# usmandroid/80211ParallelEstimation

Measured on AMD Instinct MI355X. Metric: MMSE-estimated 802.11 frames/sec (53 subcarriers) at 1/2/4/8 MI355X; % roofline, higher is better.
Workload: dtype f64; 1 GPU; PS_MMSE textbook, BASELINE configs[2]; frames_per_gpu=65536, global_frames=65536, subcarriers=53, ofdm_blocks=15, parallelism=dp1 (frames sharded, 1 RCCL state broadcast)

## Files before the change

### 80211parallelestimation_amd/csrc/wce_api.cpp

```cpp
#include <hip/hip_runtime.h>
#include <cstdio>
#include <cstring>
#include <map>
#include <memory>
#include <mutex>
#include <new>
#include <string>
#include <vector>

#include "wce_internal.h"

using wce::State;

struct wce_ctx {
    int device = 0;
    State *d_state = nullptr;
    bool ready = false;
    bool has_host = false;
    State host;
    int32_t mode = -1;
    bool fuse = true;
    bool bdot = true;
    int32_t cov_k0 = -1;
    int32_t cov_rank = 0;
    int cov_taps = 0;
    int cov_path = 0;
    int cus = 0;
    bool r1_plain = false;
    bool cm_on = false;
    bool cm_use = true;
    std::vector<wce_complex> rhh;
    std::mutex ws_mu;
    std::map<void *, std::unique_ptr<wce::Workspace>> ws_by_stream;
    int64_t ws_hint = 0;
};

static constexpr int64_t WS_LD = 64;
static constexpr int64_t WS_ARRAYS = 5;

static thread_local std::string g_err;

static bool state_r1_plain(const State *st) { return st->acoef == 1.0 && st->xmask == (1ull << wce::NSC) - 1; }

static int fail(int code, const char *what)
{
    g_err = what;
    return code;
}

static int hipfail(hipError_t e, const char *what)
{
    g_err = std::string(what) + ": " + hipGetErrorString(e);
    return WCE_EHIP;
}

#define HIPCHECK(x, what)                         \
    do {                                          \
        hipError_t e_ = (x);                      \
        if (e_ != hipSuccess) return hipfail(e_, what); \
    } while (0)
// ... 14 lines not shown
struct DeviceGuard {
    int prev = -1;
    explicit DeviceGuard(int d)
    {
        if (hipGetDevice(&prev) != hipSuccess) prev = -1;
        if (prev != d) (void)hipSetDevice(d);
    }
    ~DeviceGuard()
    {
        int cur = -1;
        if (prev >= 0 && hipGetDevice(&cur) == hipSuccess && cur != prev) (void)hipSetDevice(prev);
    }
};
}

extern "C" {

const char *wce_last_error(void) { return g_err.c_str(); }
const char *wce_version(void) { return "wce 0.1.0 (gfx950)"; }

int wce_ctx_create_empty(wce_ctx **out, int device)
{
    if (!out) return fail(WCE_EINVAL, "null ctx pointer");
    int rc = check_device(device);
    if (rc) return rc;
    wce_ctx *c = new (std::nothrow) wce_ctx();
    if (!c) return fail(WCE_ENOMEM, "ctx alloc");
    c->device = device;
    DeviceGuard g(device);
    if (hipDeviceGetAttribute(&c->cus, hipDeviceAttributeMultiprocessorCount, device) != hipSuccess || c->cus <= 0) {
        delete c;
        return fail(WCE_EHIP, "hipDeviceGetAttribute(multiprocessor count)");
    }
    hipError_t e = hipMalloc(&c->d_state, sizeof(State));
    if (e != hipSuccess) { delete c; return hipfail(e, "hipMalloc(state)"); }
    e = hipMemset(c->d_state, 0, sizeof(State));
    if (e != hipSuccess) { (void)hipFree(c->d_state); delete c; return hipfail(e, "hipMemset(state)"); }
    *out = c;
    return WCE_OK;
}

int wce_ctx_create(wce_ctx **out, int device, const wce_complex *tx_pre, const wce_complex *rx_pre, double ow2,
                   int mode)
{
    if (!out || !tx_pre || !rx_pre) return fail(WCE_EINVAL, "null argument");
    if (mode != WCE_MMSE_REF && mode != WCE_MMSE_TEXTBOOK) return fail(WCE_EINVAL, "bad mmse mode");
    if (!(ow2 > 0)) return fail(WCE_EINVAL, "ow2 must be > 0");
    wce_ctx *c = nullptr;
    int rc = wce_ctx_create_empty(&c, device);
    if (rc) return rc;
    wce::ldc txl[wce::NSC], rxl[wce::NSC], hlt[wce::NSC];
    for (int k = 0; k < wce::NSC; k++) {
        txl[k].re = tx_pre[k].re; txl[k].im = tx_pre[k].im;
        rxl[k].re = rx_pre[k].re; rxl[k].im = rx_pre[k].im;
    }
    wce::host_lt_ls(txl, rxl, hlt);
    rc = wce::host_build_state(&c->host, wce::host_reference_F(), wce::host_reference_invF(), hlt, txl, ow2, mode);
    if (rc) { wce_ctx_destroy(c); return fail(rc, "state build"); }
    c->has_host = true;
    c->mode = mode;
    c->r1_plain = state_r1_plain(&c->host);
    DeviceGuard g(device);
    hipError_t e = hipMemcpy(c->d_state, &c->host, sizeof(State), hipMemcpyHostToDevice);
    if (e != hipSuccess) { wce_ctx_destroy(c); return hipfail(e, "upload state"); }
    c->ready = true;
    *out = c;
// ... 501 lines not shown
    if (r.prep != wce::FcPrep::None) {
        rc = prep_frame_cov(c, in, out, r, sa, ws, stream);
        if (rc) return rc;
    }
    double *aux = ws ? ws + (WS_ARRAYS - 1) * n * WS_LD * 2 : nullptr;
    if (split) {
        sa.split = 1;
        if (r.form == wce::SolveForm::Bordered) {
            sa.dots = aux;
        } else {
            sa.w = ws;
            sa.ws = WS_LD;
        }
    }
    double *H = reinterpret_cast<double *>(out->ps_mmse);
    if (r.cm) {
        uint8_t *flags = reinterpret_cast<uint8_t *>(aux);
        rc = wce::launch_cm(c->d_state, sa, flags, stream);
        if (rc) return fail(rc, "constant-modulus launch");
        sa.skip = flags;
    }
    const State *st = c->d_state;
    switch (r.solve) {
    case wce::SolveStep::None: return WCE_OK;
    case wce::SolveStep::RefLsElemDone:
        rc = wce::launch_ref_ls_elem(st, sa, la, true, stream);
        return rc ? fail(rc, "ls epilogue launch") : WCE_OK;
    case wce::SolveStep::LowRank:
        rc = wce::launch_mmse_lr(st, cov_lr_k0(c), c->cov_rank, c->cov_taps, sa, stream);
        if (rc) return fail(rc, "mmse_lr launch");
        break;
    case wce::SolveStep::RefPilots: rc = wce::launch_mmse_ref_pilots(st, sa, stream); break;
    case wce::SolveStep::RefLsElem: rc = wce::launch_ref_ls_elem(st, sa, la, false, stream); break;
    case wce::SolveStep::Closed: rc = wce::launch_mmse_rank1(st, sa, false, c->cus, c->r1_plain, stream); break;
    case wce::SolveStep::ClosedNt: rc = wce::launch_mmse_rank1(st, sa, true, c->cus, c->r1_plain, stream); break;
    case wce::SolveStep::Factor: rc = wce::launch_mmse_factor(st, sa, r.form, stream); break;
    case wce::SolveStep::Fused: rc = wce::launch_mmse_solve_ls(st, sa, la, r.form, stream); break;
    }
    if (rc) return fail(rc, "mmse_solve launch");
    switch (r.finish) {
    case wce::Finish::None: break;
    case wce::Finish::AvgBlocks:
        rc = wce::launch_avg_blocks(ws, WS_LD, H, out->out_stride, n, stream);
        return rc ? fail(rc, "block average launch") : WCE_OK;
    case wce::Finish::FcFinish: rc = wce::launch_fc_finish(sa, aux, H, out->out_stride, stream); break;
    case wce::Finish::MatvecAvg:
        rc = wce::launch_matvec_avg(st->C, ws, WS_LD, sa.nblk, H, out->out_stride, n, stream);
        break;
    case wce::Finish::Apply:
        rc = wce::launch_mmse_apply(st, H, H, out->out_stride, n, stream, sa.skip);
        break;
    }
    return rc ? fail(rc, "mmse apply launch") : WCE_OK;
}

int wce_estimate(wce_ctx *c, const wce_frames *in, const wce_outputs *out, uint32_t mask, void *stream)
{
    return estimate_impl(c, in, out, mask, stream, nullptr);
}

int wce_estimate_noise(wce_ctx *c, const wce_frames *in, const wce_outputs *out, uint32_t mask, const double *ow2,
                       void *stream)
{
    return estimate_impl(c, in, out, mask, stream, nullptr, ow2);
}

struct wce_plan {
    wce_plan() = default;
// ... 535 lines not shown
```

### 80211parallelestimation_amd/csrc/wce_internal.h

```cpp
#pragma once
#include <mutex>
#include <stdint.h>
#include <stddef.h>
#include "../../include/wce.h"
#include "wce_route.h"

namespace wce {

constexpr int NSC = WCE_NSC;
constexpr int NBLK = WCE_NBLK;
constexpr int NPAD = 64;
constexpr int CLD = 64;
constexpr int PILOT[4] = {WCE_P0, WCE_P1, WCE_P2, WCE_P3};
constexpr int32_t STATE_MAGIC = 0x80211;
constexpr int32_t STATE_LAYOUT = 9;
constexpr int COV_K0_MAX = 6;

constexpr int LRL_RMAX = 8;
constexpr int LRL_NP = LRL_RMAX * (LRL_RMAX + 1) / 2;
struct State {
    double C[CLD * CLD * 2];
    double Mu[CLD * CLD * 2];
    double Wp[4 * NPAD * 2];
    double cvec[NPAD * 2];
// ... 145 lines not shown

struct ViterbiArgs {
    const float *llr;
    int64_t lfs, lbs, n;
    int32_t mod, rate, T;
    uint32_t flags;
    uint8_t *bits;
    const uint8_t *ref;
    uint32_t *nbiterr;
    int64_t bits_stride, ref_stride;
};

struct ReencodeArgs {
    const uint8_t *bits;
    const double *theta;
    const double *ptx, *rx;
    int64_t bits_stride, fs, bs, n;
    int32_t mod, rate;
    double scale, d;
    double *tx, *h;
    int64_t tfs, tbs, hs;
};

int launch_ls(const State *st, const LsArgs &a, void *stream);
int launch_demod(const DemodArgs &a, void *stream);
int launch_demap(const DemapArgs &a, void *stream);
int launch_reencode(const ReencodeArgs &a, void *stream);
int launch_viterbi(const ViterbiArgs &a, void *stream);
int decode_info_bits(int mod, int rate);
int launch_front(const FrontArgs &a, bool preamble, void *stream);
int launch_sync(const SyncArgs &a, int cus, void *stream);
int launch_mmse_ref_pilots(const State *st, const SolveArgs &a, void *stream);
int launch_mmse_factor(const State *st, const SolveArgs &a, SolveForm form, void *stream);
int launch_mmse_rank1(const State *st, const SolveArgs &a, bool nt, int cus, bool plain, void *stream);
int rank1_rows_per_sweep(int cus);
int launch_mmse_solve_ls(const State *st, const SolveArgs &a, const LsArgs &l, SolveForm form, void *stream);
int launch_ref_ls_elem(const State *st, const SolveArgs &a, const LsArgs &l, bool mmse_done, void *stream);
int launch_mmse_apply(const State *st, const double *W, double *H, int64_t stride, int64_t n, void *stream,
                      const uint8_t *skip = nullptr);
int launch_cm(const State *st, const SolveArgs &a, uint8_t *flags, void *stream);
int launch_matvec(const double *M1, const double *M2, const double *X, int64_t xs, double *Y1, double *Y2,
                  int64_t ys, int64_t n, bool qin, void *stream);
int launch_matvec_avg(const double *M, const double *X, int64_t xs, int nb, double *Y, int64_t ys, int64_t n,
                      void *stream);
int launch_fc_finish(const SolveArgs &a, const double *dots, double *H, int64_t hs, void *stream);
int launch_synth(const State *st, const SynthArgs &a, void *stream);
int launch_lr_quad2(const State *st, int rank, const SolveArgs &a, void *stream, int form = 0);
int launch_mmse_lr(const State *st, int k0, int rank, int taps, const SolveArgs &a, void *stream);
const char *lr_kernel_name(int k0, int rank, int taps, int64_t units);
int launch_ref_fc(const State *st, const SolveArgs &a, const double *rx_pre, int64_t ps, const double *tx_pre,
                  void *stream);
int launch_fc_u(const State *st, const double *rx_pre, int64_t ps, const double *tx_pre, double *U, int64_t us,
                int64_t n, void *stream);
int launch_ref_w(const State *st, const double *X, int64_t xs, double *W, int64_t ws, int64_t n, void *stream);
int launch_avg_blocks(const double *X, int64_t xs, double *H, int64_t hs, int64_t n, void *stream);
int set_flat_chunk(int64_t frames);
constexpr int WCE_VARIANT_REF = 0;
constexpr int WCE_VARIANT_LS = 1;
constexpr int WCE_VARIANT_REF_LS = 2;
constexpr int WCE_VARIANT_LR = 3;
constexpr int WCE_VARIANT_REF_FC = 4;
constexpr int WCE_VARIANT_R1 = 5;
constexpr int WCE_VARIANT_COUNT = 6;
int variant_value(int which);
int set_variant(int which, int value);
int launch_ldc_convert(const void *src, void *dst, int64_t n, bool to_complex, void *stream);
int launch_nonfinite_scan(const double *H, int64_t stride, int64_t n, bool f32, uint32_t *bits,
// ... 14 lines not shown
```

### 80211parallelestimation_amd/csrc/wce_kernels.hip

```cpp
#include <hip/hip_runtime.h>
#include "wce_internal.h"
#include "wce_device.h"

namespace wce {

constexpr int LS_WAVES = 4;
constexpr int LS_FRAMES = 4;

struct LsLane {
    double2 tpk, tden, hlt_shared;
    double cq, s0, s1, s2, s3, alpha, dk0, dk1, dk2;
    int seg;
};
__device__ __forceinline__ LsLane ls_lane(const State *__restrict__ st, const double *tx_pre, int k)
{
    LsLane c;
    const double *txp = tx_pre ? tx_pre : st->tx_pre;
    c.tpk = ld2(txp, k);
    c.cq = c.tpk.x - c.tpk.y;
    c.tden = make_double2(c.cq * c.tpk.x, c.cq * c.tpk.y);
    c.hlt_shared = ld2(st->h_lt, k);
    c.s0 = st->sinc[0][k]; c.s1 = st->sinc[1][k]; c.s2 = st->sinc[2][k]; c.s3 = st->sinc[3][k];
    c.seg = k < WCE_P1 ? 0 : (k < WCE_P2 ? 1 : 2);
    c.alpha = (double)(k - (c.seg == 0 ? WCE_P0 : (c.seg == 1 ? WCE_P1 : WCE_P2))) * (1.0 / 14.0);
// ... 2320 lines not shown
                                                             unsigned long long *n_bad)
{
    const uint32_t E = nfr * (uint32_t)NSC;
    for (uint32_t e = blockIdx.x * 256u + threadIdx.x; e < E; e += gridDim.x * 256u) {
        const uint32_t f = e / NSC, k = e - f * NSC;
        const int64_t idx = (f_begin + f) * stride + k;
        double re, im;
        if constexpr (F32) {
            const v2f t = reinterpret_cast<const v2f *>(H)[idx];
            re = t.x;
            im = t.y;
        } else {
            const double2 t = ld2(H, idx);
            re = t.x;
            im = t.y;
        }
        if (!(__builtin_isfinite(re) && __builtin_isfinite(im))) {
            const int64_t fg = f_begin + f;
            const uint32_t bit = 1u << (fg & 31);
            const uint32_t old = atomicOr(&bits[fg >> 5], bit);
            if (!(old & bit) && n_bad) atomicAdd(n_bad, 1ull);
        }
    }
}

static int hip_status(hipError_t e) { return e == hipSuccess ? WCE_OK : WCE_EHIP; }

constexpr int LR_FPW = 64;
constexpr int64_t LR_FPW_BELOW = 131072;
constexpr int64_t LR_STAGE_FROM = 0;
static int g_variant[WCE_VARIANT_COUNT] = {0, 2, 0, 0, 0, 0};
int set_variant(int which, int value)
{
    if (which < 0 || which >= WCE_VARIANT_COUNT || value < 0 || value > 15) return WCE_EINVAL;
    __atomic_store_n(&g_variant[which], value, __ATOMIC_RELAXED);
    return WCE_OK;
}
static inline int variant(int which) { return __atomic_load_n(&g_variant[which], __ATOMIC_RELAXED); }
int variant_value(int which) { return which >= 0 && which < WCE_VARIANT_COUNT ? variant(which) : 0; }

static int cu_count()
{
    constexpr int kMaxDev = 64;
    static int cache[kMaxDev] = {};
    int dev = 0;
    if (hipGetDevice(&dev) != hipSuccess || dev < 0) dev = 0;
    int *slot = dev < kMaxDev ? &cache[dev] : nullptr;
    int cus = slot ? __atomic_load_n(slot, __ATOMIC_RELAXED) : 0;
    if (cus <= 0) {
        int n = 0;
        cus = hipDeviceGetAttribute(&n, hipDeviceAttributeMultiprocessorCount, dev) == hipSuccess && n > 0 ? n : 256;
        if (slot) __atomic_store_n(slot, cus, __ATOMIC_RELAXED);
    }
    return cus;
}

static int64_t tile_blocks(int64_t tiles, int waves_per_cu)
{
    const int64_t cap = (int64_t)cu_count() * waves_per_cu / LS_WAVES;
    const int64_t need = (tiles + LS_WAVES - 1) / LS_WAVES;
    return need < cap ? need : cap;
}

int launch_ls(const State *st, const LsArgs &a, void *stream)
{
    if (a.n <= 0) return WCE_OK;
    const int64_t groups = (a.n + LS_FRAMES - 1) / LS_FRAMES;
// ... 774 lines not shown
```

### 80211parallelestimation_amd/csrc/wce_rank1.hip

```cpp
#include "wce_internal.h"
#include "wce_device.h"

namespace wce {

__device__ __forceinline__ double2 r1_mul(double2 a, double2 b)
{
#pragma clang fp contract(off)
    return make_double2(a.x * b.x - a.y * b.y, a.x * b.y + a.y * b.x);
}
__device__ __forceinline__ double2 r1_add(double2 a, double2 b)
{
#pragma clang fp contract(off)
    return make_double2(a.x + b.x, a.y + b.y);
}

__device__ __forceinline__ double2 rank1_p(double2 u, double2 w, bool cwg)
{
#pragma clang fp contract(off)
    return cwg ? r1_mul(w, u) : make_double2(u.x * u.x + u.y * u.y, 0.0);
}

template <bool PLAIN>
__device__ __forceinline__ double2 rank1_s(const double2 (&x)[4], const double2 (&r)[4], const double2 (&u)[4],
                                           const double2 (&w)[4], const double2 (&p)[4], bool cwg, double ac,
                                           double bc)
{
#pragma clang fp contract(off)
    double2 g = make_double2(0.0, 0.0), q = g;
#pragma unroll
    for (int m = 0; m < 4; ++m) {
        const double x2 = x[m].x * x[m].x + x[m].y * x[m].y;
        const double ax2 = PLAIN ? x2 : ac * x2;
        const double2 gk = make_double2(ax2 * p[m].x, ax2 * p[m].y);
        const double2 qk = r1_mul(r1_mul(w[m], cconj(x[m])), r[m]);
        g = m ? r1_add(g, gk) : gk;
        q = m ? r1_add(q, qk) : qk;
    }
    g = row16_sum(g);
    q = row16_sum(q);
    const double2 d = make_double2(bc + g.x, g.y);
    double2 t;
    if (cwg) {
        const double den = d.x * d.x + d.y * d.y;
        t = make_double2((q.x * d.x + q.y * d.y) / den, (q.y * d.x - q.x * d.y) / den);
    } else {
        t = make_double2(q.x / d.x, q.y / d.x);
    }
    double2 c = make_double2(0.0, 0.0);
#pragma unroll
    for (int m = 0; m < 4; ++m) {
        const double2 xu = r1_mul(x[m], u[m]);
        const double2 at = r1_mul(PLAIN ? xu : make_double2(ac * xu.x, ac * xu.y), t);
        const double2 rho = make_double2(r[m].x - at.x, r[m].y - at.y);
        const double ti = 2.0 * x[m].y;
        const double2 ck = r1_mul(w[m], make_double2(-(ti * rho.y), ti * rho.x));
        c = m ? r1_add(c, ck) : ck;
    }
    c = row16_sum(c);
    return make_double2(t.x + c.x / bc, t.y + c.y / bc);
}

constexpr int R1_WG_PER_CU = 4;
constexpr int R1_POL_DEFAULT = 0, R1_POL_NT = 1, R1_POL_NT_STORES = 2, R1_POL_NT_LOADS = 3;
constexpr int R1_POL_U_FIRST = 4;
constexpr int R1_POL_TX_FIRST = 5;

constexpr bool r1_prefetch(bool noise, bool shared) { return shared && !noise; }

template <int POL, bool NOISE, bool SHARED, bool SPLIT, bool PF, bool PLAIN>
__global__ __launch_bounds__(256, R1_WG_PER_CU) void mmse_rank1_kernel(const State *__restrict__ st, SolveArgs a)
{
    static_assert(!PF || r1_prefetch(NOISE, SHARED), "this instantiation has no registers for a second unit");
    constexpr bool NTL = POL == R1_POL_NT || POL == R1_POL_NT_LOADS;
    constexpr bool NTS = POL == R1_POL_NT || POL == R1_POL_NT_STORES;
    constexpr bool LF = POL != R1_POL_U_FIRST;
    constexpr bool TXF = POL == R1_POL_TX_FIRST;
    static_assert(!TXF || (SHARED && PLAIN), "the tx-first order is built for the shared-u builds without mask and scale");
    const int i = threadIdx.x & 15;
    const uint32_t rpw = blockDim.x >> 4;
    int64_t n = a.n;
    if (LF) {
        auto held = [](int64_t &c, auto v) __attribute__((always_inline)) { asm("" : "+s"(c) : "s"(v)); };
        held(n, st), held(n, a.tx), held(n, a.rx), held(n, a.fs), held(n, a.bs), held(n, a.blk), held(n, a.cu);
        held(n, rpw), held(n, gridDim.x);
        if (SPLIT) held(n, a.nblk), held(n, a.dots);
        else held(n, a.w), held(n, a.ws);
        if (NOISE) held(n, a.ow2);
        if (!SHARED) held(n, a.cs), held(n, a.cw);
    }
    const uint32_t units = (uint32_t)(SPLIT ? n * a.nblk : n);
    const uint32_t rows = gridDim.x * rpw;
    uint32_t g = blockIdx.x * rpw + (threadIdx.x >> 4);
    if (g >= units) return;
    const bool cwg = !SHARED && a.cw != nullptr;
    double ac;
    uint64_t xm;
    auto scalars = [&](double &b) __attribute__((always_inline)) {
        ac = PLAIN ? 1.0 : st->acoef;
        xm = PLAIN ? ~0ull : st->xmask;
        if (!NOISE) b = st->bcoef;
    };
    const double2 zero = make_double2(0.0, 0.0);
    auto lane_again = [](int l) __attribute__((always_inline)) {
        asm volatile("" : "+v"(l));
        return l;
    };
    auto frame_of = [&](uint32_t gu) __attribute__((always_inline)) { return SPLIT ? gu / (uint32_t)a.nblk : gu; };
    auto fetch = [&](uint32_t gu, double2(&xl)[4], double2(&rl)[4], double &bc, int part = 0) __attribute__((always_inline)) {
        const uint32_t f = frame_of(gu);
        const int b = SPLIT ? (int)(gu - f * (uint32_t)a.nblk) : 0;
        const int64_t base = (int64_t)f * a.fs + (int64_t)(a.blk + b) * a.bs + lane_again(i);
        if (TXF) {
            if (part != 2) {
#pragma unroll
                for (int m = 0; m < 3; ++m) xl[m] = ld2(a.tx, base + 16 * m);
                xl[3] = zero;
                if (i < NSC - 48) xl[3] = ld2(a.tx, base + 48);
            }
            if (part != 1) {
#pragma unroll
                for (int m = 0; m < 3; ++m) rl[m] = ld2(a.rx, base + 16 * m);
                rl[3] = zero;
                if (i < NSC - 48) rl[3] = ld2(a.rx, base + 48);
                if (NOISE) bc = a.ow2[f];
            }
            return;
        }
#pragma unroll
        for (int m = 0; m < 3; ++m) {
            xl[m] = NTL ? ld2_nt(a.tx, base + 16 * m) : ld2(a.tx, base + 16 * m);
            rl[m] = NTL ? ld2_nt(a.rx, base + 16 * m) : ld2(a.rx, base + 16 * m);
        }
        xl[3] = zero;
        rl[3] = zero;
        if (i < NSC - 48) {
            xl[3] = NTL ? ld2_nt(a.tx, base + 48) : ld2(a.tx, base + 48);
            rl[3] = NTL ? ld2_nt(a.rx, base + 48) : ld2(a.rx, base + 48);
        }
        if (NOISE) bc = a.ow2[f];
    };
    auto factors = [&](int64_t cb, double2(&u)[4], double2(&w)[4], double2(&p)[4]) __attribute__((always_inline)) {
        const int64_t ub = cb + i;
        const bool live = i < NSC - 48;
        if (SHARED) {
#pragma unroll
            for (int m = 0; m < 3; ++m) {
                u[m] = ld2(a.cu, ub + 16 * m);
                w[m] = cconj(u[m]);
            }
            u[3] = zero;
            w[3] = zero;
            if (live) {
                u[3] = ld2(a.cu, ub + 48);
                w[3] = cconj(u[3]);
            }
        } else {
#pragma unroll
            for (int m = 0; m < 3; ++m) u[m] = ld2(a.cu, ub + 16 * m);
            u[3] = zero;
            if (live) u[3] = ld2(a.cu, ub + 48);
            if (cwg) {
#pragma unroll
                for (int m = 0; m < 3; ++m) w[m] = ld2(a.cw, ub + 16 * m);
                w[3] = zero;
                if (live) w[3] = ld2(a.cw, ub + 48);
            } else {
#pragma unroll
                for (int m = 0; m < 3; ++m) w[m] = cconj(u[m]);
                w[3] = live ? cconj(u[3]) : zero;
            }
        }
#pragma unroll
        for (int m = 0; m < 4; ++m) p[m] = rank1_p(u[m], w[m], cwg);
    };
    double2 u[4], w[4], p[4];
    double2 xc[4], rc[4], xn[4], rn[4];
    double bc = 0.0, bn;
    scalars(bc);
    if (TXF) {
        fetch(g, xc, rc, bc, 1);
#pragma unroll
        for (int m = 0; m < 3; ++m) u[m] = ld2(a.cu, i + 16 * m);
        u[3] = zero;
        if (i < NSC - 48) u[3] = ld2(a.cu, i + 48);
        fetch(g, xc, rc, bc, 2);
#pragma unroll
        for (int m = 0; m < 4; ++m) {
            w[m] = m < 3 || i < NSC - 48 ? cconj(u[m]) : zero;
            p[m] = rank1_p(u[m], w[m], cwg);
        }
    } else {
        if (LF) fetch(g, xc, rc, bc);
        if (SHARED) factors(0, u, w, p);
    }
    bn = bc;
    auto trip = [&](double2(&xc)[4], double2(&rc)[4], double &bc, double2(&xn)[4], double2(&rn)[4], double &bn)
                    __attribute__((always_inline)) {
        if (!PF && !LF) fetch(g, xc, rc, bc);
        const uint32_t f = frame_of(g);
        if (!SHARED) factors((int64_t)f * a.cs, u, w, p);
        const bool more = g + rows < units;
        if (PF && more) fetch(g + rows, xn, rn, bn);
        double2 x[4];
#pragma unroll
        for (int m = 0; m < 4; ++m)
            x[m] = PLAIN || ((xm >> ((i + 16 * m) & 63)) & 1ull) ? xc[m] : zero;
        double2 pl[4];
#pragma unroll
        for (int m = 0; m < 4; ++m) {
            double2 um = u[m];
            if (PF) asm volatile("" : "+v"(um.x), "+v"(um.y));
            pl[m] = PF ? rank1_p(um, w[m], cwg) : p[m];
        }
        double2 s = rank1_s<PLAIN>(x, rc, u, w, pl, cwg, ac, bc);
        if (NOISE && !(bc > 0.0 && bc < __builtin_inf())) s = make_double2(__builtin_nan(""), __builtin_nan(""));
        if (SPLIT) {
            if (i == 0) st2(a.dots, g, s);
// ... 35 lines not shown
    dim3 g, b;
    bool pf;
};

template <int POL, bool NOISE, bool SHARED, bool PLAIN>
static void launch_r1_split(const State *st, const SolveArgs &a, const R1Shape &h, hipStream_t s)
{
    if constexpr (r1_prefetch(NOISE, SHARED)) {
        if (h.pf) {
            if (a.split) hipLaunchKernelGGL((mmse_rank1_kernel<POL, NOISE, SHARED, true, true, PLAIN>), h.g, h.b, 0, s, st, a);
            else hipLaunchKernelGGL((mmse_rank1_kernel<POL, NOISE, SHARED, false, true, PLAIN>), h.g, h.b, 0, s, st, a);
            return;
        }
    }
    if (a.split) hipLaunchKernelGGL((mmse_rank1_kernel<POL, NOISE, SHARED, true, false, PLAIN>), h.g, h.b, 0, s, st, a);
    else hipLaunchKernelGGL((mmse_rank1_kernel<POL, NOISE, SHARED, false, false, PLAIN>), h.g, h.b, 0, s, st, a);
}
template <int POL, bool PLAIN = false>
static void launch_r1_pol(const State *st, const SolveArgs &a, const R1Shape &h, hipStream_t s)
{
    const bool shared = a.cs == 0 && !a.cw;
    if constexpr (POL == R1_POL_TX_FIRST) {
        if (a.ow2) launch_r1_split<POL, true, true, PLAIN>(st, a, h, s);
        else launch_r1_split<POL, false, true, PLAIN>(st, a, h, s);
    } else if (a.ow2) {
        if (shared) launch_r1_split<POL, true, true, PLAIN>(st, a, h, s);
        else launch_r1_split<POL, true, false, PLAIN>(st, a, h, s);
    } else {
        if (shared) launch_r1_split<POL, false, true, PLAIN>(st, a, h, s);
        else launch_r1_split<POL, false, false, PLAIN>(st, a, h, s);
    }
}

int launch_mmse_rank1(const State *st, const SolveArgs &a, bool nt, int cus, bool plain, void *stream)
{
    if (!a.cu) return WCE_EINVAL;
    if (a.split ? !a.dots : !a.w) return WCE_EINVAL;
    if (a.n <= 0) return WCE_OK;
    if (a.nblk > 1 && !a.split) return WCE_EINVAL;
    if (a.ow2 && a.cw) return WCE_EINVAL;
    const int64_t units = a.split ? a.n * a.nblk : a.n;
    if (units > 0x7fffffffll) return WCE_EINVAL;
    const int shape = variant_value(WCE_VARIANT_R1);
    const int rpw = shape == 8 ? 4 : shape == 9 ? 8 : 16;
    int64_t wgs = (units + rpw - 1) / rpw;
    const bool looping = shape == 4 || shape == 7;
    const int64_t cap = shape == 4 ? 3 : shape == 7 ? rank1_rows_per_sweep(cus) / 16 : wgs;
    if (wgs > cap) wgs = cap;
    const R1Shape h{dim3((unsigned)wgs), dim3(16u * rpw), looping};
    hipStream_t s = (hipStream_t)stream;
    if (nt) launch_r1_pol<R1_POL_NT>(st, a, h, s);
    else if (shape == 5) launch_r1_pol<R1_POL_NT_STORES>(st, a, h, s);
    else if (shape == 6) launch_r1_pol<R1_POL_NT_LOADS>(st, a, h, s);
    else if (shape == 10) launch_r1_pol<R1_POL_U_FIRST>(st, a, h, s);
    else if (!plain || shape == 11) launch_r1_pol<R1_POL_DEFAULT>(st, a, h, s);
    else if (a.cs == 0 && !a.cw && shape != 12) launch_r1_pol<R1_POL_TX_FIRST, true>(st, a, h, s);
    else launch_r1_pol<R1_POL_DEFAULT, true>(st, a, h, s);
    return hipGetLastError() == hipSuccess ? WCE_OK : WCE_EHIP;
}

}
```

### 80211parallelestimation_amd/csrc/wce_route.cpp

```cpp
#include <cstring>
#include <string>

#include "wce_internal.h"
#include "wce_route.h"
#include "../../include/wce_debug.h"

namespace wce {

int check_route_facts(const RouteFacts &f)
{
    if (f.mode != WCE_MMSE_REF && f.mode != WCE_MMSE_TEXTBOOK && f.mode != WCE_MMSE_COV) return WCE_EINVAL;
    if (f.semantics != WCE_SEM_C && f.semantics != WCE_SEM_MATLAB) return WCE_EINVAL;
    if (f.mask & ~0x7Fu) return WCE_EINVAL;
    if ((f.mask & WCE_MMSE_FRAME_COV) && !(f.mask & WCE_EST_PS_MMSE)) return WCE_EINVAL;
    if (f.mode != WCE_MMSE_COV && (f.lr_k0 >= 0 || f.cm)) return WCE_EINVAL;
    if (f.noise && (f.mode != WCE_MMSE_TEXTBOOK || !(f.mask & WCE_EST_PS_MMSE))) return WCE_EINVAL;
    return WCE_OK;
}

Route plan_route(const RouteFacts &f)
{
    Route r;
    const bool ls = (f.mask & (WCE_EST_LS_ALL | WCE_EQUALIZE)) != 0;
    const bool mmse = (f.mask & WCE_EST_PS_MMSE) != 0;
// ... 50 lines not shown
    case FcPrep::None: break;
    case FcPrep::RefFc: add("ref_fc"); break;
    case FcPrep::FcU: add("fc_u"); break;
    case FcPrep::General:
        if (!r.fc_lt_ready) add("ls");
        add("matvec");
        if (r.fc_ref_w) add("ref_w");
        break;
    }
    if (r.cm) add("cm");
    switch (r.solve) {
    case SolveStep::None: break;
    case SolveStep::RefPilots: add("ref_pilots"); break;
    case SolveStep::RefLsElem: add("ref_ls_elem"); break;
    case SolveStep::RefLsElemDone: add("ref_ls_elem_done"); break;
    case SolveStep::Closed: add("mmse_rank1"); break;
    case SolveStep::ClosedNt: add("mmse_rank1_nt"); break;
    case SolveStep::Factor: add(std::string("factor_") + form[(int)r.form]); break;
    case SolveStep::Fused: add(std::string("fused_") + form[(int)r.form]); break;
    case SolveStep::LowRank: add("mmse_lr"); break;
    }
    switch (r.finish) {
    case Finish::None: break;
    case Finish::FcFinish: add("fc_finish"); break;
    case Finish::MatvecAvg: add("matvec_avg"); break;
    case Finish::Apply: add("apply"); break;
    case Finish::AvgBlocks: add("avg_blocks"); break;
    }
    if (s.size() + 1 > cap || !buf) return -1;
    std::memcpy(buf, s.c_str(), s.size() + 1);
    return (int)s.size();
}

}

extern "C" int wce_debug_route(int mode, int bdot, int fuse, int cm, int lr_k0, int cov_rank, int semantics,
                               unsigned mask, int ls_f32, int r1, int ref_fc, int ref_ls, char *buf, size_t cap)
{
    const wce::RouteFacts f{mode, bdot != 0, fuse != 0, cm != 0, lr_k0, cov_rank, semantics, mask, ls_f32 != 0, r1, ref_fc, ref_ls};
    if (wce::check_route_facts(f)) return WCE_EINVAL;
    return wce::route_names(wce::plan_route(f), buf, cap) < 0 ? WCE_EINVAL : WCE_OK;
}

extern "C" int wce_debug_route_noise(int mode, int bdot, int fuse, int cm, int lr_k0, int cov_rank, int semantics,
                                     unsigned mask, int ls_f32, int r1, int ref_fc, int ref_ls, int noise, char *buf,
                                     size_t cap)
{
    wce::RouteFacts f{mode, bdot != 0, fuse != 0, cm != 0, lr_k0, cov_rank, semantics, mask, ls_f32 != 0, r1, ref_fc, ref_ls};
    f.noise = noise != 0;
    if (wce::check_route_facts(f)) return WCE_EINVAL;
    return wce::route_names(wce::plan_route(f), buf, cap) < 0 ? WCE_EINVAL : WCE_OK;
}
```

### 80211parallelestimation_amd/csrc/wce_route.h

```cpp
#pragma once
#include <cstddef>
#include <cstdint>

namespace wce {

struct RouteFacts {
    int mode;
    bool bdot;
    bool fuse;
    bool cm;
    int lr_k0;
    int cov_rank;
    int semantics;
    uint32_t mask;
    bool ls_f32;
    int r1, ref_fc, ref_ls;
    bool noise;
};

enum class FcPrep : uint8_t {
    None,
    RefFc,
    FcU,
    General,
// ... 5 lines not shown
    Dense,
};

enum class SolveStep : uint8_t {
    None,
    RefPilots,
    RefLsElem,
    RefLsElemDone,
    Closed,
    ClosedNt,
    Factor,
    Fused,
    LowRank,
};

enum class Finish : uint8_t { None, FcFinish, MatvecAvg, Apply, AvgBlocks };

struct Route {
    bool ls_pass = false;
    FcPrep prep = FcPrep::None;
    bool fc_lt_ready = false;
    bool fc_ref_w = false;
    bool cm = false;
    SolveStep solve = SolveStep::None;
    SolveForm form = SolveForm::Dense;
    Finish finish = Finish::None;
    bool workspace = false;
};

int check_route_facts(const RouteFacts &f);
Route plan_route(const RouteFacts &f);
int route_names(const Route &r, char *buf, size_t cap);

}
```

### 80211parallelestimation_amd/wce.py

```python
from __future__ import annotations

import ctypes
import os
from ctypes import POINTER, byref, c_double, c_int, c_int32, c_int64, c_size_t, c_uint32, c_uint64, c_void_p

import numpy as np

NSC = 53
NBLK = 15
DC = 26
PILOTS = (5, 19, 33, 47)

LT_LS = 1 << 0
PS_LINEAR = 1 << 1
PS_CUBIC = 1 << 2
PS_SINC = 1 << 3
PS_MMSE = 1 << 4
EQUALIZE = 1 << 5
LS_ALL = 0xF
ALL = 0x3F
OUT_LS_F32 = 1
FRAME_COV = 1 << 6

MMSE_REF = 0
# ... 55 lines not shown
    _fields_ = [("eq", c_void_p), ("sym", c_void_p), ("theta", c_void_p), ("evm", c_void_p), ("nerr", c_void_p),
                ("eq_frame_stride", c_int64), ("eq_block_stride", c_int64), ("sym_frame_stride", c_int64),
                ("sym_block_stride", c_int64)]


class ReencodePar(ctypes.Structure):
    _fields_ = [("bits", c_void_p), ("bits_stride", c_int64), ("modulation", c_int32), ("rate", c_int32),
                ("scale", c_double), ("theta", c_void_p)]


class ReencodeOut(ctypes.Structure):
    _fields_ = [("tx", c_void_p), ("tx_frame_stride", c_int64), ("tx_block_stride", c_int64), ("h", c_void_p),
                ("h_stride", c_int64)]


_lib = None

ABI = {
    "wce_ctx_create": [POINTER(c_void_p), c_int, c_void_p, c_void_p, c_double, c_int],
    "wce_ctx_create_empty": [POINTER(c_void_p), c_int],
    "wce_ctx_destroy": [c_void_p],
    "wce_ctx_reserve": [c_void_p, c_int64],
    "wce_ctx_reserve_stream": [c_void_p, c_int64, c_void_p],
    "wce_plan_create": [POINTER(c_void_p), c_void_p, c_void_p, c_void_p, c_uint32],
    "wce_plan_launch": [c_void_p, c_void_p],
    "wce_plan_destroy": [c_void_p],
    "wce_ctx_create_cov": [POINTER(c_void_p), c_int, c_void_p, c_void_p, c_void_p, c_double],
    "wce_state_build_cov": [c_void_p, c_size_t, c_void_p, c_void_p, c_void_p, c_double],
    "wce_debug_set_fusion": [c_void_p, c_int],
    "wce_debug_set_border_dot": [c_void_p, c_int],
    "wce_debug_set_flat_chunk": [ctypes.c_int64],
    "wce_debug_set_variant": [c_int, c_int],
    "wce_debug_rank1_rows_per_sweep": [c_void_p],
    "wce_debug_set_cov_path": [c_void_p, c_int],
    "wce_debug_lr_kernel": [c_void_p, c_int64],
    "wce_debug_route": [c_int] * 7 + [c_uint32] + [c_int] * 4 + [ctypes.c_char_p, c_size_t],
    "wce_debug_route_noise": [c_int] * 7 + [c_uint32] + [c_int] * 5 + [ctypes.c_char_p, c_size_t],
    "wce_debug_cov_factor": [c_void_p, c_size_t, c_void_p, POINTER(c_int), POINTER(c_int), POINTER(c_double),
                             POINTER(c_double)],
    "wce_ctx_cov_info": [c_void_p, POINTER(c_int), POINTER(c_int), POINTER(c_double), POINTER(c_double)],
    "wce_ctx_set_modulus": [c_void_p, c_void_p],
    "wce_state_set_modulus": [c_void_p, c_size_t, c_void_p, c_void_p],
    "wce_debug_set_cm": [c_void_p, c_int],
    "wce_debug_compat_state_builds": [],
    "wce_ctx_state": [c_void_p, POINTER(c_void_p), POINTER(c_size_t)],
    "wce_ctx_mark_ready": [c_void_p],
    "wce_state_size": [],
    "wce_state_build": [c_void_p, c_size_t, c_void_p, c_void_p, c_double, c_int],
    "wce_ctx_load_state": [c_void_p, c_void_p, c_size_t],
    "wce_state_validate": [c_void_p, c_size_t, POINTER(c_int)],
    "wce_ctx_get_shared": [c_void_p, c_void_p, c_void_p, POINTER(c_double), POINTER(c_double)],
    "wce_estimate": [c_void_p, POINTER(Frames), POINTER(Outputs), c_uint32, c_void_p],
    "wce_estimate_noise": [c_void_p, POINTER(Frames), POINTER(Outputs), c_uint32, c_void_p, c_void_p],
    "wce_mmse_solve": [c_void_p, POINTER(Frames), c_void_p, c_int64, c_void_p],
    "wce_mmse_apply": [c_void_p, c_void_p, c_void_p, c_int64, c_int64, c_void_p],
    "wce_synth_frames": [c_void_p, c_void_p, c_void_p, c_void_p, c_int64, c_int64, c_int64, c_int64, c_int64,
                         c_uint64, c_void_p, c_double, c_double, c_void_p],
    "wce_front_end_blocks": [c_void_p, c_void_p, c_int64, c_int64, c_int32, c_void_p, c_int64, c_int64, c_void_p],
    "wce_front_end_preamble": [c_void_p, c_void_p, c_int64, c_int64, c_int64, c_void_p, c_int64, c_void_p,
                               c_void_p],
    "wce_front_end_blocks_cfo": [c_void_p, c_void_p, c_int64, c_int64, c_int32, c_void_p, c_int64, c_void_p, c_int64,
                                 c_int64, c_void_p],
    "wce_front_end_preamble_cfo": [c_void_p, c_void_p, c_int64, c_int64, c_int64, c_void_p, c_int64, c_void_p,
                                   c_void_p, c_int, c_void_p],
    "wce_front_end_sync": [c_void_p, c_void_p, c_int64, c_int64, c_int64, c_void_p, c_double, c_int32, c_void_p,
                           c_void_p, c_void_p],
# ... 857 lines not shown
```

### include/wce_debug.h

```cpp
#ifndef WCE_DEBUG_H
#define WCE_DEBUG_H
#include <stddef.h>
#ifdef __cplusplus
extern "C" {
#endif
int wce_debug_reference_F(long double *out);
int wce_debug_reference_invF(long double *out);
int wce_debug_build_state(const double *tx_pre, const double *rx_pre, double ow2, int mode, double *C,
                          double *h_lt, double *sinc, double *ab, unsigned long long *xmask);
int wce_debug_cov_factor(const void *blob, size_t bytes, double *U, int *rank, int *k0, double *lmax, double *lmin);
struct wce_ctx;
int wce_debug_set_fusion(struct wce_ctx *ctx, int on);
int wce_debug_set_border_dot(struct wce_ctx *ctx, int on);
int wce_debug_set_flat_chunk(long long frames);
int wce_debug_set_variant(int which, int value);
int wce_debug_rank1_rows_per_sweep(struct wce_ctx *ctx);
int wce_debug_route(int mode, int bdot, int fuse, int cm, int lr_k0, int cov_rank, int semantics, unsigned mask,
                    int ls_f32, int r1, int ref_fc, int ref_ls, char *buf, size_t cap);
int wce_debug_route_noise(int mode, int bdot, int fuse, int cm, int lr_k0, int cov_rank, int semantics,
                          unsigned mask, int ls_f32, int r1, int ref_fc, int ref_ls, int noise, char *buf,
                          size_t cap);
int wce_debug_set_cov_path(struct wce_ctx *ctx, int path);
const char *wce_debug_lr_kernel(struct wce_ctx *ctx, long long units);
int wce_debug_set_cm(struct wce_ctx *ctx, int on);
unsigned long long wce_debug_compat_state_builds(void);
#ifdef __cplusplus
}
#endif
#endif
```

Measured before the change: 2.302 billion frames/s.

## Add specialized rank-1 MMSE head kernel with XCD-aware workgroup remapping

New measurement: 2.376 billion frames/s (median of 6 runs). 3.2% higher.

```diff
diff --git a/80211parallelestimation_amd/csrc/wce_api.cpp b/80211parallelestimation_amd/csrc/wce_api.cpp
--- a/80211parallelestimation_amd/csrc/wce_api.cpp
+++ b/80211parallelestimation_amd/csrc/wce_api.cpp
@@ -26,6 +26,7 @@
     int cov_taps = 0;
     int cov_path = 0;
     int cus = 0;
+    int xcds = 1;
     bool r1_plain = false;
     bool cm_on = false;
     bool cm_use = true;
@@ -106,6 +107,12 @@
         delete c;
         return fail(WCE_EHIP, "hipDeviceGetAttribute(multiprocessor count)");
     }
+    hipDeviceProp_t prop;
+    if (hipGetDeviceProperties(&prop, device) != hipSuccess) {
+        delete c;
+        return fail(WCE_EHIP, "hipGetDeviceProperties");
+    }
+    c->xcds = std::strncmp(prop.gcnArchName, "gfx950", 6) == 0 ? wce::R1_HEAD_XCDS : 1;
     hipError_t e = hipMalloc(&c->d_state, sizeof(State));
     if (e != hipSuccess) { delete c; return hipfail(e, "hipMalloc(state)"); }
     e = hipMemset(c->d_state, 0, sizeof(State));
@@ -673,8 +680,8 @@
         break;
     case wce::SolveStep::RefPilots: rc = wce::launch_mmse_ref_pilots(st, sa, stream); break;
     case wce::SolveStep::RefLsElem: rc = wce::launch_ref_ls_elem(st, sa, la, false, stream); break;
-    case wce::SolveStep::Closed: rc = wce::launch_mmse_rank1(st, sa, false, c->cus, c->r1_plain, stream); break;
-    case wce::SolveStep::ClosedNt: rc = wce::launch_mmse_rank1(st, sa, true, c->cus, c->r1_plain, stream); break;
+    case wce::SolveStep::Closed: rc = wce::launch_mmse_rank1(st, sa, false, c->cus, c->xcds, c->r1_plain, stream); break;
+    case wce::SolveStep::ClosedNt: rc = wce::launch_mmse_rank1(st, sa, true, c->cus, c->xcds, c->r1_plain, stream); break;
     case wce::SolveStep::Factor: rc = wce::launch_mmse_factor(st, sa, r.form, stream); break;
     case wce::SolveStep::Fused: rc = wce::launch_mmse_solve_ls(st, sa, la, r.form, stream); break;
     }
diff --git a/80211parallelestimation_amd/csrc/wce_internal.h b/80211parallelestimation_amd/csrc/wce_internal.h
--- a/80211parallelestimation_amd/csrc/wce_internal.h
+++ b/80211parallelestimation_amd/csrc/wce_internal.h
@@ -201,7 +201,7 @@
 int launch_sync(const SyncArgs &a, int cus, void *stream);
 int launch_mmse_ref_pilots(const State *st, const SolveArgs &a, void *stream);
 int launch_mmse_factor(const State *st, const SolveArgs &a, SolveForm form, void *stream);
-int launch_mmse_rank1(const State *st, const SolveArgs &a, bool nt, int cus, bool plain, void *stream);
+int launch_mmse_rank1(const State *st, const SolveArgs &a, bool nt, int cus, int nx, bool plain, void *stream);
 int rank1_rows_per_sweep(int cus);
 int launch_mmse_solve_ls(const State *st, const SolveArgs &a, const LsArgs &l, SolveForm form, void *stream);
 int launch_ref_ls_elem(const State *st, const SolveArgs &a, const LsArgs &l, bool mmse_done, void *stream);
diff --git a/80211parallelestimation_amd/csrc/wce_kernels.hip b/80211parallelestimation_amd/csrc/wce_kernels.hip
--- a/80211parallelestimation_amd/csrc/wce_kernels.hip
+++ b/80211parallelestimation_amd/csrc/wce_kernels.hip
@@ -2376,7 +2376,7 @@
 static int g_variant[WCE_VARIANT_COUNT] = {0, 2, 0, 0, 0, 0};
 int set_variant(int which, int value)
 {
-    if (which < 0 || which >= WCE_VARIANT_COUNT || value < 0 || value > 15) return WCE_EINVAL;
+    if (which < 0 || which >= WCE_VARIANT_COUNT || value < 0 || value > 31) return WCE_EINVAL;
     __atomic_store_n(&g_variant[which], value, __ATOMIC_RELAXED);
     return WCE_OK;
 }
diff --git a/80211parallelestimation_amd/csrc/wce_rank1.hip b/80211parallelestimation_amd/csrc/wce_rank1.hip
--- a/80211parallelestimation_amd/csrc/wce_rank1.hip
+++ b/80211parallelestimation_amd/csrc/wce_rank1.hip
@@ -1,66 +1,7 @@
-#include "wce_internal.h"
-#include "wce_device.h"
+#include "wce_rank1_body.h"
 
 namespace wce {
 
-__device__ __forceinline__ double2 r1_mul(double2 a, double2 b)
-{
-#pragma clang fp contract(off)
-    return make_double2(a.x * b.x - a.y * b.y, a.x * b.y + a.y * b.x);
-}
-__device__ __forceinline__ double2 r1_add(double2 a, double2 b)
-{
-#pragma clang fp contract(off)
-    return make_double2(a.x + b.x, a.y + b.y);
-}
-
-__device__ __forceinline__ double2 rank1_p(double2 u, double2 w, bool cwg)
-{
-#pragma clang fp contract(off)
-    return cwg ? r1_mul(w, u) : make_double2(u.x * u.x + u.y * u.y, 0.0);
-}
-
-template <bool PLAIN>
-__device__ __forceinline__ double2 rank1_s(const double2 (&x)[4], const double2 (&r)[4], const double2 (&u)[4],
-                                           const double2 (&w)[4], const double2 (&p)[4], bool cwg, double ac,
-                                           double bc)
-{
-#pragma clang fp contract(off)
-    double2 g = make_double2(0.0, 0.0), q = g;
-#pragma unroll
-    for (int m = 0; m < 4; ++m) {
-        const double x2 = x[m].x * x[m].x + x[m].y * x[m].y;
-        const double ax2 = PLAIN ? x2 : ac * x2;
-        const double2 gk = make_double2(ax2 * p[m].x, ax2 * p[m].y);
-        const double2 qk = r1_mul(r1_mul(w[m], cconj(x[m])), r[m]);
-        g = m ? r1_add(g, gk) : gk;
-        q = m ? r1_add(q, qk) : qk;
-    }
-    g = row16_sum(g);
-    q = row16_sum(q);
-    const double2 d = make_double2(bc + g.x, g.y);
-    double2 t;
-    if (cwg) {
-        const double den = d.x * d.x + d.y * d.y;
-        t = make_double2((q.x * d.x + q.y * d.y) / den, (q.y * d.x - q.x * d.y) / den);
-    } else {
-        t = make_double2(q.x / d.x, q.y / d.x);
-    }
-    double2 c = make_double2(0.0, 0.0);
-#pragma unroll
-    for (int m = 0; m < 4; ++m) {
-        const double2 xu = r1_mul(x[m], u[m]);
-        const double2 at = r1_mul(PLAIN ? xu : make_double2(ac * xu.x, ac * xu.y), t);
-        const double2 rho = make_double2(r[m].x - at.x, r[m].y - at.y);
-        const double ti = 2.0 * x[m].y;
-        const double2 ck = r1_mul(w[m], make_double2(-(ti * rho.y), ti * rho.x));
-        c = m ? r1_add(c, ck) : ck;
-    }
-    c = row16_sum(c);
-    return make_double2(t.x + c.x / bc, t.y + c.y / bc);
-}
-
-constexpr int R1_WG_PER_CU = 4;
 constexpr int R1_POL_DEFAULT = 0, R1_POL_NT = 1, R1_POL_NT_STORES = 2, R1_POL_NT_LOADS = 3;
 constexpr int R1_POL_U_FIRST = 4;
 constexpr int R1_POL_TX_FIRST = 5;
@@ -111,17 +52,9 @@
         const int b = SPLIT ? (int)(gu - f * (uint32_t)a.nblk) : 0;
         const int64_t base = (int64_t)f * a.fs + (int64_t)(a.blk + b) * a.bs + lane_again(i);
         if (TXF) {
-            if (part != 2) {
-#pragma unroll
-                for (int m = 0; m < 3; ++m) xl[m] = ld2(a.tx, base + 16 * m);
-                xl[3] = zero;
-                if (i < NSC - 48) xl[3] = ld2(a.tx, base + 48);
-            }
+            if (part != 2) r1_fetch_row(a.tx, base, i, xl);
             if (part != 1) {
-#pragma unroll
-                for (int m = 0; m < 3; ++m) rl[m] = ld2(a.rx, base + 16 * m);
-                rl[3] = zero;
-                if (i < NSC - 48) rl[3] = ld2(a.rx, base + 48);
+                r1_fetch_row(a.rx, base, i, rl);
                 if (NOISE) bc = a.ow2[f];
             }
             return;
@@ -179,10 +112,7 @@
     scalars(bc);
     if (TXF) {
         fetch(g, xc, rc, bc, 1);
-#pragma unroll
-        for (int m = 0; m < 3; ++m) u[m] = ld2(a.cu, i + 16 * m);
-        u[3] = zero;
-        if (i < NSC - 48) u[3] = ld2(a.cu, i + 48);
+        r1_fetch_row(a.cu, i, i, u);
         fetch(g, xc, rc, bc, 2);
 #pragma unroll
         for (int m = 0; m < 4; ++m) {
@@ -284,7 +214,9 @@
     }
 }
 
-int launch_mmse_rank1(const State *st, const SolveArgs &a, bool nt, int cus, bool plain, void *stream)
+void launch_mmse_rank1_head(const State *st, const SolveArgs &a, const R1HeadShape &h, void *stream);
+
+int launch_mmse_rank1(const State *st, const SolveArgs &a, bool nt, int cus, int nx, bool plain, void *stream)
 {
     if (!a.cu) return WCE_EINVAL;
     if (a.split ? !a.dots : !a.w) return WCE_EINVAL;
@@ -294,6 +226,12 @@
     const int64_t units = a.split ? a.n * a.nblk : a.n;
     if (units > 0x7fffffffll) return WCE_EINVAL;
     const int shape = variant_value(WCE_VARIANT_R1);
+    const R1HeadShape head = rank1_head_shape(
+        R1HeadFacts{a.cs == 0 && !a.cw, a.split != 0, a.ow2 != nullptr, a.cw != nullptr, plain, nt, shape, a.fs, a.ws, a.n}, nx);
+    if (head.threads) {
+        launch_mmse_rank1_head(st, a, head, stream);
+        return hipGetLastError() == hipSuccess ? WCE_OK : WCE_EHIP;
+    }
     const int rpw = shape == 8 ? 4 : shape == 9 ? 8 : 16;
     int64_t wgs = (units + rpw - 1) / rpw;
     const bool looping = shape == 4 || shape == 7;
diff --git a/80211parallelestimation_amd/csrc/wce_rank1_body.h b/80211parallelestimation_amd/csrc/wce_rank1_body.h
--- /dev/null
+++ b/80211parallelestimation_amd/csrc/wce_rank1_body.h
@@ -0,0 +1,74 @@
+#pragma once
+#include "wce_internal.h"
+#include "wce_device.h"
+
+namespace wce {
+
+__device__ __forceinline__ double2 r1_mul(double2 a, double2 b)
+{
+#pragma clang fp contract(off)
+    return make_double2(a.x * b.x - a.y * b.y, a.x * b.y + a.y * b.x);
+}
+__device__ __forceinline__ double2 r1_add(double2 a, double2 b)
+{
+#pragma clang fp contract(off)
+    return make_double2(a.x + b.x, a.y + b.y);
+}
+
+__device__ __forceinline__ double2 rank1_p(double2 u, double2 w, bool cwg)
+{
+#pragma clang fp contract(off)
+    return cwg ? r1_mul(w, u) : make_double2(u.x * u.x + u.y * u.y, 0.0);
+}
+
+template <bool PLAIN>
+__device__ __forceinline__ double2 rank1_s(const double2 (&x)[4], const double2 (&r)[4], const double2 (&u)[4],
+                                           const double2 (&w)[4], const double2 (&p)[4], bool cwg, double ac,
+                                           double bc)
+{
+#pragma clang fp contract(off)
+    double2 g = make_double2(0.0, 0.0), q = g;
+#pragma unroll
+    for (int m = 0; m < 4; ++m) {
+        const double x2 = x[m].x * x[m].x + x[m].y * x[m].y;
+        const double ax2 = PLAIN ? x2 : ac * x2;
+        const double2 gk = make_double2(ax2 * p[m].x, ax2 * p[m].y);
+        const double2 qk = r1_mul(r1_mul(w[m], cconj(x[m])), r[m]);
+        g = m ? r1_add(g, gk) : gk;
+        q = m ? r1_add(q, qk) : qk;
+    }
+    g = row16_sum(g);
+    q = row16_sum(q);
+    const double2 d = make_double2(bc + g.x, g.y);
+    double2 t;
+    if (cwg) {
+        const double den = d.x * d.x + d.y * d.y;
+        t = make_double2((q.x * d.x + q.y * d.y) / den, (q.y * d.x - q.x * d.y) / den);
+    } else {
+        t = make_double2(q.x / d.x, q.y / d.x);
+    }
+    double2 c = make_double2(0.0, 0.0);
+#pragma unroll
+    for (int m = 0; m < 4; ++m) {
+        const double2 xu = r1_mul(x[m], u[m]);
+        const double2 at = r1_mul(PLAIN ? xu : make_double2(ac * xu.x, ac * xu.y), t);
+        const double2 rho = make_double2(r[m].x - at.x, r[m].y - at.y);
+        const double ti = 2.0 * x[m].y;
+        const double2 ck = r1_mul(w[m], make_double2(-(ti * rho.y), ti * rho.x));
+        c = m ? r1_add(c, ck) : ck;
+    }
+    c = row16_sum(c);
+    return make_double2(t.x + c.x / bc, t.y + c.y / bc);
+}
+
+__device__ __forceinline__ void r1_fetch_row(const double *p, int64_t base, int i, double2 (&v)[4])
+{
+#pragma unroll
+    for (int m = 0; m < 3; ++m) v[m] = ld2(p, base + 16 * m);
+    v[3] = make_double2(0.0, 0.0);
+    if (i < NSC - 48) v[3] = ld2(p, base + 48);
+}
+
+constexpr int R1_WG_PER_CU = 4;
+
+}
diff --git a/80211parallelestimation_amd/csrc/wce_rank1_head.hip b/80211parallelestimation_amd/csrc/wce_rank1_head.hip
--- /dev/null
+++ b/80211parallelestimation_amd/csrc/wce_rank1_head.hip
@@ -0,0 +1,66 @@
+#include "wce_rank1_body.h"
+
+namespace wce {
+
+template <int T, bool XCD8>
+__global__ __launch_bounds__(T, R1_WG_PER_CU) void mmse_rank1_head_kernel(const State *st, const double *tx,
+                                                                          const double *rx, const double *cu,
+                                                                          double *H, uint32_t n, uint32_t fs,
+                                                                          uint32_t ws)
+{
+    static_assert(T == 64 || T == 128 || T == 256, "whole waves, at most mmse_rank1_kernel's workgroup");
+    constexpr uint32_t RPW = T / 16;
+    const int i = threadIdx.x & 15;
+    constexpr uint32_t NX = R1_HEAD_XCDS;
+    uint32_t wg = blockIdx.x;
+    if (XCD8) {
+        const uint32_t groups = (n + RPW - 1) / RPW;
+        wg = rank1_head_group(wg, NX, (groups + NX - 1) / NX);
+        if (wg >= groups) return;
+    }
+    const uint32_t g = wg * RPW + (threadIdx.x >> 4);
+    if (g >= n) return;
+    const double bc = st->bcoef;
+    double2 x[4], r[4], u[4], w[4], p[4];
+    const int64_t base = (int64_t)((uint64_t)g * fs) + i;
+    r1_fetch_row(tx, base, i, x);
+    r1_fetch_row(cu, i, i, u);
+    r1_fetch_row(rx, base, i, r);
+#pragma unroll
+    for (int m = 0; m < 4; ++m) {
+        w[m] = m < 3 || i < NSC - 48 ? cconj(u[m]) : make_double2(0.0, 0.0);
+        p[m] = rank1_p(u[m], w[m], false);
+    }
+    const double2 s = rank1_s<true>(x, r, u, w, p, false, 1.0, bc);
+    const int64_t hb = (int64_t)((uint64_t)g * ws) + i;
+#pragma unroll
+    for (int m = 0; m < 4; ++m)
+        if (i + 16 * m < NSC) st2(H, hb + 16 * m, r1_mul(u[m], s));
+}
+
+template <int T>
+static void launch_head(const State *st, const SolveArgs &a, bool remap, hipStream_t s)
+{
+    constexpr int64_t RPW = T / 16;
+    const int64_t groups = (a.n + RPW - 1) / RPW;
+    const double *tx = a.tx + 2 * ((int64_t)a.blk * a.bs), *rx = a.rx + 2 * ((int64_t)a.blk * a.bs);
+    const uint32_t n = (uint32_t)a.n, fs = (uint32_t)a.fs, ws = (uint32_t)a.ws;
+    if (remap) {
+        const int64_t per = (groups + R1_HEAD_XCDS - 1) / R1_HEAD_XCDS;
+        hipLaunchKernelGGL((mmse_rank1_head_kernel<T, true>), dim3((unsigned)(R1_HEAD_XCDS * per)), dim3(T), 0, s, st, tx, rx,
+                           a.cu, a.w, n, fs, ws);
+    } else {
+        hipLaunchKernelGGL((mmse_rank1_head_kernel<T, false>), dim3((unsigned)groups), dim3(T), 0, s, st, tx, rx,
+                           a.cu, a.w, n, fs, ws);
+    }
+}
+
+void launch_mmse_rank1_head(const State *st, const SolveArgs &a, const R1HeadShape &h, void *stream)
+{
+    hipStream_t s = (hipStream_t)stream;
+    if (h.threads == 64) launch_head<64>(st, a, h.remap, s);
+    else if (h.threads == 128) launch_head<128>(st, a, h.remap, s);
+    else launch_head<256>(st, a, h.remap, s);
+}
+
+}
diff --git a/80211parallelestimation_amd/csrc/wce_route.cpp b/80211parallelestimation_amd/csrc/wce_route.cpp
--- a/80211parallelestimation_amd/csrc/wce_route.cpp
+++ b/80211parallelestimation_amd/csrc/wce_route.cpp
@@ -106,6 +106,35 @@
     return (int)s.size();
 }
 
+R1HeadShape rank1_head_shape(const R1HeadFacts &f, int nx)
+{
+    const R1HeadShape old{0, false};
+    if (!f.shared || f.split || f.noise || f.cw || !f.plain || f.nt) return old;
+    if (f.fs < 0 || f.fs > 0xffffffffll || f.ws < 0 || f.ws > 0xffffffffll || f.n > 0x7fffffffll) return old;
+    const int v = f.variant == 0 ? R1_VARIANT_ADOPTED : f.variant;
+    if (v < R1_VARIANT_HEAD_FIRST || v > R1_VARIANT_HEAD_LAST) return old;
+    const int k = (v - R1_VARIANT_HEAD_FIRST) % 3;
+    return R1HeadShape{64 << k, v >= R1_VARIANT_HEAD_FIRST + 3 && nx == R1_HEAD_XCDS};
+}
+
+}
+
+extern "C" int wce_debug_rank1_head(int shared, int split, int noise, int cw, int plain, int nt, int variant,
+                                    long long fs, long long ws, long long n, int nx, int *remap)
+{
+    const wce::R1HeadFacts f{shared != 0, split != 0, noise != 0, cw != 0, plain != 0, nt != 0, variant, fs, ws, n};
+    const wce::R1HeadShape h = wce::rank1_head_shape(f, nx);
+    if (remap) *remap = h.remap;
+    return h.threads;
+}
+
+extern "C" int wce_debug_rank1_head_groups(unsigned groups, unsigned nx, unsigned *out, unsigned cap)
+{
+    if (!groups || !nx || groups > 0x7fffffffu || nx > 64) return WCE_EINVAL;
+    const unsigned per = (groups + nx - 1) / nx, grid = nx * per;
+    if (!out || cap < grid) return WCE_EINVAL;
+    for (unsigned b = 0; b < grid; b++) out[b] = wce::rank1_head_group(b, nx, per);
+    return (int)grid;
 }
 
 extern "C" int wce_debug_route(int mode, int bdot, int fuse, int cm, int lr_k0, int cov_rank, int semantics,
diff --git a/80211parallelestimation_amd/csrc/wce_route.h b/80211parallelestimation_amd/csrc/wce_route.h
--- a/80211parallelestimation_amd/csrc/wce_route.h
+++ b/80211parallelestimation_amd/csrc/wce_route.h
@@ -61,4 +61,28 @@
 Route plan_route(const RouteFacts &f);
 int route_names(const Route &r, char *buf, size_t cap);
 
+struct R1HeadFacts {
+    bool shared;
+    bool split;
+    bool noise;
+    bool cw;
+    bool plain;
+    bool nt;
+    int variant;
+    int64_t fs, ws, n;
+};
+struct R1HeadShape {
+    int threads;
+    bool remap;
+};
+constexpr int R1_VARIANT_HEAD_OFF = 13, R1_VARIANT_HEAD_FIRST = 14, R1_VARIANT_HEAD_LAST = 19;
+constexpr int R1_VARIANT_ADOPTED = 18;
+constexpr int R1_HEAD_XCDS = 8;
+R1HeadShape rank1_head_shape(const R1HeadFacts &f, int nx);
+
+#ifdef __HIPCC__
+__host__ __device__
+#endif
+inline uint32_t rank1_head_group(uint32_t b, uint32_t nx, uint32_t per) { return (b % nx) * per + b / nx; }
+
 }
diff --git a/80211parallelestimation_amd/wce.py b/80211parallelestimation_amd/wce.py
--- a/80211parallelestimation_amd/wce.py
+++ b/80211parallelestimation_amd/wce.py
@@ -111,6 +111,8 @@
     "wce_debug_set_flat_chunk": [ctypes.c_int64],
     "wce_debug_set_variant": [c_int, c_int],
     "wce_debug_rank1_rows_per_sweep": [c_void_p],
+    "wce_debug_rank1_head": [c_int] * 7 + [c_int64] * 3 + [c_int, POINTER(c_int)],
+    "wce_debug_rank1_head_groups": [c_uint32, c_uint32, POINTER(c_uint32), c_uint32],
     "wce_debug_set_cov_path": [c_void_p, c_int],
     "wce_debug_lr_kernel": [c_void_p, c_int64],
     "wce_debug_route": [c_int] * 7 + [c_uint32] + [c_int] * 4 + [ctypes.c_char_p, c_size_t],
diff --git a/include/wce_debug.h b/include/wce_debug.h
--- a/include/wce_debug.h
+++ b/include/wce_debug.h
@@ -15,6 +15,9 @@
 int wce_debug_set_flat_chunk(long long frames);
 int wce_debug_set_variant(int which, int value);
 int wce_debug_rank1_rows_per_sweep(struct wce_ctx *ctx);
+int wce_debug_rank1_head(int shared, int split, int noise, int cw, int plain, int nt, int variant, long long fs,
+                         long long ws, long long n, int nx, int *remap);
+int wce_debug_rank1_head_groups(unsigned groups, unsigned nx, unsigned *out, unsigned cap);
 int wce_debug_route(int mode, int bdot, int fuse, int cm, int lr_k0, int cov_rank, int semantics, unsigned mask,
                     int ls_f32, int r1, int ref_fc, int ref_ls, char *buf, size_t cap);
 int wce_debug_route_noise(int mode, int bdot, int fuse, int cm, int lr_k0, int cov_rank, int semantics,
```
